# zchuning/repo

Hardware: AMD Instinct MI355X
Metric: world-model+imagine updates/sec (B=50,L=50,64x64x3) (higher is better)
Workload: dtype f32

## Files before the change

### repo_amd/csrc/conv.hip

```cpp
#include <stdlib.h>

#include <algorithm>
#include <type_traits>

#include "igemm.h"
#include "dconv.h"
#include "uconv.h"
#include "dconv_up.h"
#include "bconv.h"
#include "buconv.h"
#include "bwgrad.h"
#include "bdec4.h"
#include "twgrad.h"
#include "tconv_up.h"
#include "tconv_down.h"


namespace repo {

static thread_local int t_bconv_enabled = 1;

template <int CB_, int CS_, int HB_, int KS_>
struct Geo {
  static constexpr int CB = CB_, CS = CS_, HB = HB_, WB = HB_, KS = KS_;
// ... 201 lines not shown
  __shared__ float red[16][64];
  const int total = Mrows * (Ncols + 1) + (tkk > 0 ? 2 * tcb : 0);
  const int o = threadIdx.x & 63, gw = threadIdx.x >> 6;
  const int i = blockIdx.x * 64 + o;
  for (int g = gw; g < 16; g += SLAB_REDUCE_WAVES) {
    float s0 = 0.f, s1 = 0.f, s2 = 0.f, s3 = 0.f;
    if (i < total) {
      int z = g;
      for (; z + 48 < splits; z += 64) {
        s0 += slab[(size_t)z * total + i];
        s1 += slab[(size_t)(z + 16) * total + i];
        s2 += slab[(size_t)(z + 32) * total + i];
        s3 += slab[(size_t)(z + 48) * total + i];
      }
      for (; z < splits; z += 16) s0 += slab[(size_t)z * total + i];
    }
    red[g][o] = (s0 + s1) + (s2 + s3);
  }
  __syncthreads();
  const int g = gw;
  if (g == 0 && i < total) {
    float s = 0.f;
#pragma unroll
    for (int q = 0; q < 16; ++q) s += red[q][o];
    int m = i / (Ncols + 1), n = i % (Ncols + 1);
    if (tkk > 0) {
      const int body = Mrows * Ncols;
      if (i >= body + Mrows) {
        const int c = i - body - Mrows;
        if (dbig && c < tcb) {
          float s2 = 0.f;
#pragma unroll
          for (int q = 0; q < 16; ++q) s2 += red[q][o + tcb];
          dbig[c] = accumulate ? dbig[c] + (s + s2) : s + s2;
        }
        return;
      }
      if (i < body) m = (i / tcb) % Mrows, n = (i % tcb) * tkk + i / (tcb * Mrows);
      else m = i - body, n = Ncols;
    }
    if (n < Ncols) {
      float* p = dw + (size_t)m * Ncols + n;
      *p = accumulate ? *p + s : s;
    } else if (db) {
      db[m] = accumulate ? db[m] + s : s;
    }
  }
}

__global__ void partial_sum_rows_kernel(const float* __restrict__ parts, int n, float* __restrict__ out, float scale,
                                        int accumulate) {
  __shared__ float red[16];
  const float* row = parts + (size_t)blockIdx.x * n;
  float s = 0.f;
  for (int i = threadIdx.x; i < n; i += blockDim.x) s += row[i];
  s = block_sum(s, red);
  if (threadIdx.x == 0) out[blockIdx.x] = accumulate ? out[blockIdx.x] + scale * s : scale * s;
}

__global__ void partial_sum_kernel(const float* __restrict__ parts, int n, float* __restrict__ out, int accumulate) {
  __shared__ float red[16];
  float s = 0.f;
  for (int i = threadIdx.x; i < n; i += blockDim.x) s += parts[i];
  s = block_sum(s, red);
  if (threadIdx.x == 0) *out = accumulate ? *out + s : s;
}

__global__ void channel_sum_kernel(const float* __restrict__ x, int nimg, int C, int P, int imgs_per_split,
                                   float* __restrict__ parts) {
  __shared__ float red[16];
  const int c = blockIdx.x, s = blockIdx.y;
  const int i0 = s * imgs_per_split, i1 = min(nimg, i0 + imgs_per_split);
  const int nt = blockDim.x;
  const int dq = nt / P, dr = nt % P;
  int img = i0 + (int)threadIdx.x / P, p = (int)threadIdx.x % P;
  float a0 = 0.f, a1 = 0.f;
  const size_t cstride = (size_t)C * P;
  const float* base = x + (size_t)c * P;
  while (img < i1) {
    a0 += base[img * cstride + p];
    p += dr;
    img += dq;
    if (p >= P) {
      p -= P;
      ++img;
    }
    if (img >= i1) break;
    a1 += base[img * cstride + p];
    p += dr;
    img += dq;
    if (p >= P) {
      p -= P;
      ++img;
    }
  }
  const float acc = block_sum(a0 + a1, red);
  if (threadIdx.x == 0) parts[s * C + c] = acc;
}
__global__ void channel_sum_final_kernel(const float* __restrict__ parts, int splits, int C, float* __restrict__ out,
                                         int accumulate) {
  const int lane = threadIdx.x & 63;
  const int c = blockIdx.x * (blockDim.x >> 6) + (threadIdx.x >> 6);
  if (c >= C) return;
  float s = 0.f;
  for (int z = lane; z < splits; z += 64) s += parts[z * C + c];
  s = wave_sum(s);
  if (lane == 0) out[c] = accumulate ? out[c] + s : s;
}

__global__ void relu_mask_kernel(int64_t n, const float* __restrict__ dy, const float* __restrict__ h,
                                 float* __restrict__ y) {
  const int64_t stride = (int64_t)gridDim.x * blockDim.x;
  for (int64_t i = (int64_t)blockIdx.x * blockDim.x + threadIdx.x; i < n; i += stride) y[i] = h[i] > 0.f ? dy[i] : 0.f;
}

template <class G>
struct DTileFor;
template <> struct DTileFor<GEnc1> { using Down = DTile<32, 512, 3, 1, 8>; using Wgrad = WTile<32, 64, 1, 2, 1, 4, 2>; static constexpr int WGT = 3072; };
template <> struct DTileFor<GEnc2> { using Down = DTile<64, 128, 2, 2, 2>; using Wgrad = WTile<64, 128, 2, 2, 1, 7, 2>; static constexpr int WGT = 768; };
template <> struct DTileFor<GEnc3> { using Down = DTile<128, 128, 2, 2, 2>; using Wgrad = WTile<64, 128, 2, 2, 2, 6>; static constexpr int WGT = 1024; };
template <> struct DTileFor<GEnc4> { using Down = DTile<32, 64, 2, 1, 2>; using Wgrad = WTile<64, 128, 2, 2, 8, 2>; static constexpr int WGT = 768; };
template <> struct DTileFor<GDec2> { using Down = DTile<128, 128, 4, 2, 4, 1>; using Wgrad = WTile<64, 128, 2, 2, 4, 5>; static constexpr int WGT = 1536; };
template <> struct DTileFor<GDec3> { using Down = DTile<64, 128, 2, 2, 2>; using Wgrad = WTile<64, 128, 2, 2, 1, 7>; static constexpr int WGT = 2048; };
template <> struct DTileFor<GDec4> { using Down = DTile<32, 256, 3, 1, 8>; using Wgrad = WTile<32, 128, 1, 4, 1, 2>; static constexpr int WGT = 1536; };
template <> struct DTileFor<GX1> { using Down = DTile<32, 512, 3, 1, 8>;  using Wgrad = WTile<32, 64, 1, 2, 1, 2, 2>; static constexpr int WGT = 3072; };
template <> struct DTileFor<GX2> { using Down = DTile<64, 128, 2, 2, 2>;  using Wgrad = WTile<64, 128, 2, 2, 1, 3, 2>; static constexpr int WGT = 1536; };
template <> struct DTileFor<GX3> { using Down = DTile<128, 128, 2, 2, 2>; using Wgrad = WTile<64, 128, 2, 2, 1, 7>; static constexpr int WGT = 1024; };
template <> struct DTileFor<GX4> { using Down = DTile<64, 128, 2, 2, 2>;  using Wgrad = WTile<64, 128, 2, 2, 2, 6>; static constexpr int WGT = 1024; };
template <> struct DTileFor<GY4> { using Down = DTile<32, 256, 2, 1, 4>;  using Wgrad = WTile<32, 128, 1, 4, 1, 2>; static constexpr int WGT = 1536; };
template <> struct DTileFor<GT4> { using Down = DTile<32, 256, 3, 1, 8>;  using Wgrad = WTile<32, 128, 1, 4, 1, 2>; static constexpr int WGT = 1536; };
template <> struct DTileFor<GY5> { using Down = DTile<32, 512, 3, 1, 8>;  using Wgrad = WTile<32, 64, 1, 2, 1, 2>; static constexpr int WGT = 1536; };

template <class G> struct DLatTile { using type = typename DTileFor<G>::Down; };
template <> struct DLatTile<GEnc2> { using type = DTile<32, 128, 4, 1, 4>; };
template <> struct DLatTile<GEnc3> { using type = DTile<32, 128, 8, 1, 4>; };
template <> struct DLatTile<GEnc4> { using type = DTile<32, 128, 8, 1, 4>; };

struct NoBTile {};
template <class G> struct BDownFor { using type = NoBTile; };
template <> struct BDownFor<GDec3> { using type = BTile<64, 256, 2, 1, 4>; };
template <> struct BDownFor<GEnc3> { using type = BTile<128, 128, 4, 2, 2>; };
template <> struct BDownFor<GEnc4> { using type = BTile<128, 64, 4, 2, 2>; };
template <> struct BDownFor<GEnc2> { using type = BTile<64, 256, 4, 1, 4>; };
template <> struct BDownFor<GDec2> { using type = BTile<64, 128, 2, 1, 4>; };
template <class G> constexpr bool kBDown = !std::is_same<typename BDownFor<G>::type, NoBTile>::value;
template <class G> struct BDownU8For { using type = NoBTile; };
template <> struct BDownU8For<GEnc1> { using type = BTile<32, 512, 4, 1, 8>; };
template <class G> constexpr bool kBDownU8 = !std::is_same<typename BDownU8For<G>::type, NoBTile>::value;
template <class G, class BigT>
constexpr bool kBDownT = std::is_same<BigT, float>::value ? kBDown<G> : kBDownU8<G>;
template <class G, class BigT>
using BDownTile = typename std::conditional<std::is_same<BigT, float>::value, typename BDownFor<G>::type, typename BDownU8For<G>::type>::type;

template <class G, class BigT = float>
static bool bconv_down_on(int64_t nimg) {
  if constexpr (kBDownT<G, BigT>) return t_bconv_enabled && nimg * (int64_t)G::PS > 512;
  return false;
}
template <class G, class BigT = float>
static size_t bconv_pack_bytes() {
  if constexpr (kBDownT<G, BigT>) {
    typedef BPack<G, BDownTile<G, BigT>> P;
    return ((std::is_same<BigT, float>::value ? P::BYTES : P::BYTES_U8) + 255) & ~(size_t)255;
  }
  return 0;
}

template <class G, class BigT = float>
static long conv_down_tiles(int64_t nimg) {
  const long px = nimg * (long)G::PS;
  long bn = px <= 512 ? DLatTile<G>::type::BN : DTileFor<G>::Down::BN;
  if constexpr (kBDownT<G, BigT>)
    if (bconv_down_on<G, BigT>(nimg)) bn = BDownTile<G, BigT>::BN;
  return (px + bn - 1) / bn;
}

template <class G, class BigT>
static int conv_down_t(int64_t nimg, const BigT* big, const float* w, const float* bias, float* small, int epi,
                       const float* aux, float* dbias, int accumulate_dbias, unsigned char* cmask, void* ws,
                       size_t ws_bytes, hipStream_t s) {
  if (cmask && G::CS % 4 != 0) return REPO_E_BADARG;
  if (nimg * (int64_t)G::CB * G::PB >= kMaxBufElems || nimg * (int64_t)G::CS * G::PS >= kMaxBufElems) return REPO_E_SHAPE;
  bool bf = false;
  size_t pack_bytes = 0;
  if constexpr (kBDownT<G, BigT>) {
    pack_bytes = bconv_pack_bytes<G, BigT>();
    bf = bconv_down_on<G, BigT>(nimg) && ws && ws_bytes >= pack_bytes + (dbias ? (size_t)conv_down_tiles<G, BigT>(nimg) * G::CS * sizeof(float) : 0);
    if (!bf) pack_bytes = 0;
  }
  long tiles = conv_down_tiles<G, BigT>(nimg);
  if constexpr (kBDownT<G, BigT>)
    if (!bf && bconv_down_on<G, BigT>(nimg)) {
      const long px = nimg * (long)G::PS;
      tiles = (px + DTileFor<G>::Down::BN - 1) / DTileFor<G>::Down::BN;
    }
  if (dbias && (!ws || ws_bytes < pack_bytes + (size_t)tiles * G::CS * sizeof(float))) return REPO_E_WS_TOO_SMALL;
  float* parts = dbias ? (float*)((char*)ws + pack_bytes) : nullptr;
  DownArgs a{big, w, bias, aux, small, (int)nimg, epi, (unsigned)(nimg * G::CB * G::PB * sizeof(BigT)),
             (unsigned)(G::CS * G::CB * G::KK * sizeof(float)), parts, cmask};
  int rc;
#ifndef TCD_DISABLE
  if constexpr (std::is_same<G, GDec3>::value && std::is_same<BigT, float>::value) {
    if (bf && (epi == REPO_EPI_NONE || epi == REPO_EPI_MUL_DRELU) && !bias && !dbias && !cmask && nimg >= 32 &&
        pack_bytes >= TcdGeo::PACK_BYTES)
      return launch_tconv_down<TcdGeo>(a, w, (char*)ws, s);
  }
#ifndef TCD_NO_ENC2
  if constexpr (std::is_same<G, GEnc2>::value && std::is_same<BigT, float>::value) {
    if (bf && epi == REPO_EPI_RELU && !dbias && nimg >= 32 && pack_bytes >= TcdGeoE2::PACK_BYTES)
      return launch_tconv_down<TcdGeoE2>(a, w, (char*)ws, s);
  }
#endif
#endif
  if constexpr (kBDownT<G, BigT>) {
    if (bf) rc = launch_bconv_down<G, BDownTile<G, BigT>, BigT>(a, w, (char*)ws, s);
    else rc = (nimg * (int64_t)G::PS <= 512) ? launch_dconv_down<G, BigT, typename DLatTile<G>::type>(a, s)
                                            : launch_dconv_down<G, BigT, typename DTileFor<G>::Down>(a, s);
  } else {
    rc = (nimg * (int64_t)G::PS <= 512) ? launch_dconv_down<G, BigT, typename DLatTile<G>::type>(a, s)
                                        : launch_dconv_down<G, BigT, typename DTileFor<G>::Down>(a, s);
  }
  if (rc || !dbias) return rc;
  hipLaunchKernelGGL(channel_sum_final_kernel, dim3(cdiv(G::CS, 4)), dim3(256), 0, s, (const float*)parts, (int)tiles,
                     (int)G::CS, dbias, accumulate_dbias);
  REPO_CHECK_LAUNCH();
  return REPO_OK;
}

template <class G> struct UConf { using type = void; };
template <> struct UConf<GDec3> { using type = SConf<GDec3, 1, 6>; };
template <> struct UConf<GEnc2> { using type = SConf<GEnc2, 1, 8>; };
template <> struct UConf<GDec2> { using type = SConf<GDec2, 5, 2>; };
template <> struct UConf<GEnc3> { using type = SConf<GEnc3, 4, 2>; };
template <> struct UConf<GEnc4> { using type = SConf<GEnc4, 8, 1>; };
template <> struct UConf<GX3> { using type = SConf<GX3, 1, 2>; };
template <> struct UConf<GX4> { using type = SConf<GX4, 4, 1>; };

struct NoTile {};
template <class G> struct UpDirect { using type = NoTile; };
template <> struct UpDirect<GEnc2> { using type = NoTile; };
template <> struct UpDirect<GEnc3> { using type = NoTile; };
template <> struct UpDirect<GEnc4> { using type = NoTile; };
template <> struct UpDirect<GDec2> { using type = NoTile; };
template <> struct UpDirect<GDec3> { using type = NoTile; };
template <> struct UpDirect<GX2> { using type = DTile<128, 128, 8, 2, 4>; };
template <> struct UpDirect<GX3> { using type = NoTile; };
template <> struct UpDirect<GX4> { using type = NoTile; };
template <> struct UpDirect<GY4> { using type = DTile<64, 256, 4, 2, 4>; };
template <> struct UpDirect<GT4> { using type = DTile<32, 256, 4, 1, 8>; };
template <class G> constexpr bool kUpDirect = !std::is_same<typename UpDirect<G>::type, NoTile>::value;

template <class G> struct BUConf { using type = void; };
template <> struct BUConf<GDec3> { using type = BSConf<GDec3, 1, 4>; };
template <> struct BUConf<GEnc2> { using type = BSConf<GEnc2, 1, 4>; };
template <> struct BUConf<GEnc3> { using type = BSConf<GEnc3, 4, 4>; };
template <> struct BUConf<GEnc4> { using type = BSConf<GEnc4, 8, 2>; };
template <> struct BUConf<GDec2> { using type = BSConf<GDec2, 5, 4>; };
template <class G>
static bool buconv_on() {
  if constexpr (!std::is_void<typename BUConf<G>::type>::value) return t_bconv_enabled != 0;
  return false;
}

template <class G>
static size_t conv_up_ws_scatter() {
  using C = typename UConf<G>::type;
  using BC = typename BUConf<G>::type;
  if constexpr (kUpDirect<G>) return UpGeo<G>::PACK_FLOATS * sizeof(float);
  else if constexpr (std::is_void<C>::value) return 0;
  else if constexpr (!std::is_void<BC>::value) return BC::PACK_BYTES > C::PACK_FLOATS * sizeof(float) ? BC::PACK_BYTES : C::PACK_FLOATS * sizeof(float);
  else return C::PACK_FLOATS * sizeof(float);
}
template <class G> constexpr bool kTconvUp = false;
#ifndef TCU_DISABLE
template <> constexpr bool kTconvUp<GEnc2> = true;
#endif
template <class G>
static size_t conv_up_tcu_off() { return (conv_up_ws_scatter<G>() + 255) & ~(size_t)255; }
template <class G>
static size_t conv_up_ws_bytes() {
  if constexpr (kTconvUp<G>) return conv_up_tcu_off<G>() + kTcuPackBytes;
  return conv_up_ws_scatter<G>();
}

template <class G>
static int conv_up_pack_t(const float* w, void* ws, size_t ws_bytes, hipStream_t s) {
  using UC = typename UConf<G>::type;
  using BC = typename BUConf<G>::type;
  if constexpr (kTconvUp<G>) {
    if (buconv_on<G>()) {
      if (!ws || ws_bytes < conv_up_ws_bytes<G>()) return REPO_E_WS_TOO_SMALL;
      const int rc = launch_tconv_up_pack(w, (char*)ws + conv_up_tcu_off<G>(), s);
      if (rc) return rc;
    }
  }
  if constexpr (!std::is_void<BC>::value)
    if (buconv_on<G>()) return launch_buconv_pack<G, BC>(w, ws, ws_bytes, s);
  if constexpr (kUpDirect<G>) return launch_dconv_up_pack<G>(w, ws, ws_bytes, s);
  else if constexpr (!std::is_void<UC>::value) return launch_uconv_pack<G, UC>(w, ws, ws_bytes, s);
  else return REPO_OK;
}

template <class G>
static int conv_up_t(int64_t nimg, const float* small, const float* w, const float* bias, float* big, int epi,
                     const float* aux, int packed, void* ws, size_t ws_bytes, hipStream_t s) {
  if (nimg * (int64_t)G::CB * G::PB >= kMaxBufElems || nimg * (int64_t)G::CS * G::PS >= kMaxBufElems) return REPO_E_SHAPE;
  using UC = typename UConf<G>::type;
  using BC = typename BUConf<G>::type;
  if (epi == REPO_EPI_MUL_CMASK && (kUpDirect<G> || std::is_void<UC>::value || G::CB % 4 != 0)) return REPO_E_BADARG;
  if (epi == REPO_EPI_FILM_RELU && (kUpDirect<G> || std::is_void<UC>::value)) return REPO_E_BADARG;
  if constexpr (kTconvUp<G>) {
    const bool epi_ok = epi == REPO_EPI_NONE || epi == REPO_EPI_MUL_DRELU || epi == REPO_EPI_MUL_CMASK;
    if (buconv_on<G>() && epi_ok && nimg >= 4 && ws && ws_bytes >= conv_up_ws_bytes<G>()) {
      char* pack = (char*)ws + conv_up_tcu_off<G>();
      if (!packed) {
        const int rc = launch_tconv_up_pack(w, pack, s);
        if (rc) return rc;
      }
      return launch_tconv_up(small, pack, bias, aux, big, nimg, epi, s);
    }
  }
  if constexpr (!std::is_void<BC>::value)
    if (buconv_on<G>()) return launch_buconv_scatter<G, BC>(small, w, bias, aux, big, nimg, epi, packed, ws, ws_bytes, s);
  if constexpr (kUpDirect<G>) {
    return launch_dconv_up<G, typename UpDirect<G>::type>(small, w, bias, aux, big, nimg, epi, packed, ws, ws_bytes, s);
  } else if constexpr (!std::is_void<UC>::value) {
    return launch_uconv_scatter<G, UC>(small, w, bias, aux, big, nimg, epi, packed, ws, ws_bytes, s);
  } else {
    static_assert(G::KS % 2 == 0, "the gather engine pairs horizontally adjacent output pixels");
    ConvUpMergedOp<G, float, 0> op{small, w, bias, aux, big, (int)nimg, epi, nullptr, nullptr, nullptr, 0.f, 0.f};
    if constexpr (G::CB < 8) return launch_igemm<T32x256>(op, 4 * G::CB, nimg * (int64_t)op.NY * op.NX, 1, s);
    else return launch_igemm<T64x128>(op, 4 * G::CB, nimg * (int64_t)op.NY * op.NX, 1, s);
  }
}

template <class G>
static int dwgrad_ips(int64_t nimg) {
  using T = typename DTileFor<G>::Wgrad;
  const long tiles = ((G::CS + T::BM - 1) / T::BM) * ((G::CB * G::KK + T::BN - 1) / T::BN);
  long want = (DTileFor<G>::WGT + tiles - 1) / tiles;
  long ips = (nimg + want - 1) / want;
  const long min_ips = T::GI * ((G::PS >= 512) ? 1 : (G::PS >= 64 ? 2 : 4));
  if (ips < min_ips) ips = min_ips;
  ips = (ips + T::GI - 1) / T::GI * T::GI;
  return (int)ips;
}
template <class G>
static int dwgrad_splits(int64_t nimg) {
  const long ips = dwgrad_ips<G>(nimg);
  return (int)((nimg + ips - 1) / ips);
}
template <class G>
static size_t wgrad_ws_bytes(int64_t nimg) {
  return (size_t)dwgrad_splits<G>(nimg) * G::CS * (G::CB * G::KK + 1) * sizeof(float);
}

static void launch_conv_slab_reduce(const float* ws, int splits, int cs, int nw, float* dw, float* db, int accumulate,
                                    hipStream_t s) {
  const int total = cs * (nw + 1);
  if (splits >= 64 && total <= 65536) {
    hipLaunchKernelGGL(conv_slab_reduce_wave_kernel, dim3(cdiv(total, 64)), dim3(64 * SLAB_REDUCE_WAVES), 0, s, ws, splits, cs, nw, dw, db,
                       accumulate, 0, 0, (float*)nullptr);
  } else {
// ... 345 lines not shown
```

### repo_amd/csrc/tconv_down.h

```cpp
#pragma once
#include "bgemm.h"
#include "dconv.h"
#include "twgrad.h"

namespace repo {

template <int KS_, int WB_, int WS_, int GST_, int NTL_>
struct TcdGeoT {
  static constexpr int CB = 32, CS = 64, WB = WB_, HB = WB_, WS = WS_, PS = WS_ * WS_, PB = WB_ * WB_, KS = KS_, KK = KS_ * KS_;
  static_assert(KS % 2 == 0 && WS == (WB - KS) / 2 + 1 && HB <= 32, "even kernel, stride 2, at most 32 rows (the staging items)");
  static constexpr int CC = 8;
  static constexpr int NCH = CB / CC;
  static constexpr int NST = KK / 4;
  static constexpr int GST = GST_, NGR = NST / GST;
  static constexpr int XH = (WB + 1) / 2, PIXB = 16;
  static constexpr int PO = 256, ROWB = PO + XH * PIXB;
  static_assert(XH * PIXB <= PO, "a column-parity plane of a row fits 256 B");
  static constexpr int KP = KS / 2;
  static constexpr int tap_of(int s, int kg) { return ((2 * s + (kg >> 1)) / KP) * KS + 2 * ((2 * s + (kg >> 1)) % KP) + (kg & 1); }
  static constexpr int SLOTSTEP = (2 * ROWB / PIXB) % 16;
  static constexpr int PPLANE = HB * ROWB, PBUF = 3 * PPLANE;
  static constexpr int WPL = CS * 4 * 16;
  static constexpr int WSTEP = 3 * WPL, WGRP = GST * WSTEP;
  static constexpr int LDS_BYTES = 2 * PBUF + 2 * WGRP;
  static constexpr int NTL = NTL_;
  static constexpr int W_PER = WGRP / 16 / 256;
  static constexpr int QPR = (WB + 3) / 4, P_PER = 2;
  static_assert(WGRP % (16 * 256) == 0 && QPR == 8 && NST % GST == 0 && NCH % 2 == 0 && NGR <= 3 && NGR >= P_PER, "staging shares");
  static constexpr size_t PACK_BYTES = (size_t)NCH * NST * WSTEP;
};
using TcdGeo = TcdGeoT<6, 30, 13, 3, 6>;
using TcdGeoE2 = TcdGeoT<4, 31, 14, 2, 7>;
constexpr size_t kTcdPackBytes = TcdGeo::PACK_BYTES;

template <class T>
__global__ __launch_bounds__(256) void tconv_down_pack_kernel(const float* w, char* pack) {
  const int i = blockIdx.x * 256 + threadIdx.x;
  if (i >= T::NCH * T::NST * T::CS * 4) return;
  const int kg = i & 3, cs = (i >> 2) % T::CS, st = (i >> 2) / T::CS;
  const int c = st / T::NST, tap = T::tap_of(st % T::NST, kg);
  float v[8];
#pragma unroll
  for (int j = 0; j < 8; ++j) v[j] = w[((size_t)cs * T::CB + T::CC * c + j) * T::KK + tap];
  unsigned pl[3][4];
#pragma unroll
  for (int e = 0; e < 4; ++e) bg_split3(v[2 * e], v[2 * e + 1], pl[0][e], pl[1][e], pl[2][e]);
  char* dst = pack + (size_t)st * T::WSTEP + ((cs >> 4) * 64 + kg * 16 + (cs & 15)) * 16;
#pragma unroll
  for (int q = 0; q < 3; ++q) *reinterpret_cast<u32x4s*>(dst + q * T::WPL) = u32x4s{pl[q][0], pl[q][1], pl[q][2], pl[q][3]};
}

template <class T, int KEPI>
__global__ __launch_bounds__(512) void tconv_down_kernel(DownArgs p) {
  extern __shared__ __attribute__((aligned(16))) char td_lds[];
  char* const Pb = td_lds;
  char* const Wr = td_lds + 2 * T::PBUF;
  const int tid = threadIdx.x;
  const int wid = __builtin_amdgcn_readfirstlane(tid >> 6);
  const int nloc = (p.nimg - (int)blockIdx.x + (int)gridDim.x - 1) / (int)gridDim.x;
  if (nloc <= 0) return;
  const int nchunks = nloc * T::NCH;

  if (wid < 4) {
    __builtin_amdgcn_s_setprio(2);
    const int lane = tid & 63;
    const int mh = wid & 1, nh = wid >> 1;
    const int ln = lane & 15, kg = lane >> 4;
    int pxs[T::NTL], pfirst = 0;
#pragma unroll
    for (int t = 0; t < T::NTL; ++t) pxs[t] = -1;
    {
      int cnt = 0;
#pragma unroll
      for (int sy = T::WS - 1; sy >= 0; --sy) {
        const int sx = (ln - T::SLOTSTEP * sy) & 15;
        if (sx < T::WS) pfirst = T::WS * sy + sx;
      }
#pragma unroll
      for (int sy = 0; sy < T::WS; ++sy) {
        const int sx = (ln - T::SLOTSTEP * sy) & 15;
        const int idx = cnt - T::NTL * nh;
#pragma unroll
        for (int t = 0; t < T::NTL; ++t)
          if (sx < T::WS && idx == t) pxs[t] = T::WS * sy + sx;
        cnt += sx < T::WS ? 1 : 0;
      }
    }
    int nbase[T::NTL];
#pragma unroll
    for (int t = 0; t < T::NTL; ++t) {
      const int px = pxs[t] < 0 ? pfirst : pxs[t];
      const int sy = px / T::WS, sx = px - sy * T::WS;
      nbase[t] = 2 * sy * T::ROWB + sx * T::PIXB;
    }
    int toff[T::NST];
#pragma unroll
    for (int s = 0; s < T::NST; ++s) {
      const int pr = 2 * s + (kg >> 1), ky = pr / T::KP, kx = 2 * (pr - T::KP * ky) + (kg & 1);
      toff[s] = ky * T::ROWB + (kx & 1) * T::PO + (kx >> 1) * T::PIXB;
    }
    const int abase = 2 * mh * 1024 + lane * 16;

    f32x4 acc[2][T::NTL];
#pragma unroll
    for (int m = 0; m < 2; ++m)
#pragma unroll
      for (int t = 0; t < T::NTL; ++t) acc[m][t] = f32x4{0.f, 0.f, 0.f, 0.f};

    const __amdgpu_buffer_rsrc_t rout = make_rsrc(p.out, 4u * (unsigned)p.nimg * T::CS * T::PS);
    const __amdgpu_buffer_rsrc_t raux = make_rsrc(KEPI == REPO_EPI_MUL_DRELU ? p.aux : p.out, 4u * (unsigned)p.nimg * T::CS * T::PS);

    unsigned eoff[T::NTL];
#pragma unroll
    for (int t = 0; t < T::NTL; ++t) {
      eoff[t] = (4u * (unsigned)((32 * mh + 4 * kg) * T::PS + max(pxs[t], 0))) | ((unsigned)(pxs[t] >> 31) & kOobOffset);
    }
    float av[2][T::NTL][4];
    float bv[2][4];
#pragma unroll
    for (int m = 0; m < 2; ++m)
#pragma unroll
      for (int r = 0; r < 4; ++r) bv[m][r] = (KEPI == REPO_EPI_RELU && p.bias) ? p.bias[32 * mh + 16 * m + 4 * kg + r] : 0.f;

    lds_barrier();
    int ph = 0;
    for (int cc = 0; cc < nchunks; ++cc) {
      const char* Pl = Pb + (cc & 1) * T::PBUF;
      const unsigned ibase = 4u * (unsigned)(((int)blockIdx.x + (cc / T::NCH) * (int)gridDim.x) * T::CS * T::PS);
      if (KEPI == REPO_EPI_MUL_DRELU && (cc & (T::NCH - 1)) == T::NCH - 1) {
#pragma unroll
        for (int t = 0; t < T::NTL; ++t)
#pragma unroll
          for (int m = 0; m < 2; ++m)
#pragma unroll
            for (int r = 0; r < 4; ++r)
              av[m][t][r] = __builtin_bit_cast(float, __builtin_amdgcn_raw_buffer_load_b32(raux, eoff[t] + ibase + 4u * (unsigned)((16 * m + r) * T::PS), 0, 0));
      }
      bg_bf16x8 fa[2][2][3], fb[3][3];
#pragma unroll
      for (int g = 0; g < T::NGR; ++g) {
        const char* Wl = Wr + (ph & 1) * T::WGRP;
        auto load_a = [&](bg_bf16x8(&fa)[2][3], int k) __attribute__((always_inline)) {
#pragma unroll
          for (int m = 0; m < 2; ++m)
#pragma unroll
            for (int q = 0; q < 3; ++q)
              fa[m][q] = *reinterpret_cast<const bg_bf16x8*>(Wl + k * T::WSTEP + q * T::WPL + abase + m * 1024);
        };
        auto load_b = [&](bg_bf16x8(&fb)[3], int s, int t) __attribute__((always_inline)) {
#pragma unroll
          for (int q = 0; q < 3; ++q) fb[q] = *reinterpret_cast<const bg_bf16x8*>(Pl + q * T::PPLANE + nbase[t] + toff[s]);
        };
        load_a(fa[0], 0);
        if (g == 0) {
          load_b(fb[0], 0, 0);
          load_b(fb[1], 0, 1);
        }
        constexpr int NIT = T::GST * T::NTL;
#pragma unroll
        for (int it = 0; it < NIT; ++it) {
          const int k = it / T::NTL, t = it % T::NTL;
          if (it + 2 < NIT) load_b(fb[(it + 2) % 3], g * T::GST + (it + 2) / T::NTL, (it + 2) % T::NTL);
          if (t == 0 && k + 1 < T::GST) load_a(fa[(k + 1) & 1], k + 1);
          __builtin_amdgcn_sched_barrier(0);
          constexpr int PA[6] = {1, 0, 2, 0, 1, 0}, PB[6] = {1, 2, 0, 1, 0, 0};
#pragma unroll
          for (int pr = 0; pr < 6; ++pr)
#pragma unroll
            for (int m = 0; m < 2; ++m)
#ifdef TCD_NO_MFMA
              acc[m][t][0] += __builtin_bit_cast(float, (int)fa[k & 1][m][PA[pr]][0] + (int)fb[it % 3][PB[pr]][0]);
#else
              acc[m][t] = __builtin_amdgcn_mfma_f32_16x16x32_bf16(fa[k & 1][m][PA[pr]], fb[it % 3][PB[pr]], acc[m][t], 0, 0, 0);
#endif
          __builtin_amdgcn_sched_barrier(0);
        }
        if (g + 1 < T::NGR) {
          load_b(fb[0], (g + 1) * T::GST, 0);
          load_b(fb[1], (g + 1) * T::GST, 1);
        }
        lds_barrier();
        ++ph;
      }
#ifndef TCD_NO_EPI
      if ((cc & (T::NCH - 1)) == T::NCH - 1)
#else
      if (cc == nchunks - 1)
#endif
      {
        const int img = (int)blockIdx.x + (cc / T::NCH) * (int)gridDim.x;
#pragma unroll
        for (int t = 0; t < T::NTL; ++t)
#pragma unroll
          for (int m = 0; m < 2; ++m) {
            unsigned bits = 0;
#pragma unroll
            for (int r = 0; r < 4; ++r) {
              float x = acc[m][t][r];
              if (KEPI == REPO_EPI_MUL_DRELU) x = av[m][t][r] > 0.f ? x : 0.f;
              if (KEPI == REPO_EPI_RELU) {
                x = fmaxf(x + bv[m][r], 0.f);
                bits |= (x > 0.f ? 1u : 0u) << r;
              }
              __builtin_amdgcn_raw_buffer_store_b32(__builtin_bit_cast(unsigned, x), rout, eoff[t] + ibase + 4u * (unsigned)((16 * m + r) * T::PS), 0, 0);
              acc[m][t][r] = 0.f;
            }
            if (KEPI == REPO_EPI_RELU && p.cmask && pxs[t] >= 0)
              p.cmask[((size_t)img * (T::CS / 4) + 8 * mh + 4 * m + kg) * T::PS + pxs[t]] = (unsigned char)bits;
          }
      }
    }
  } else {
    const int t_ = tid - 256;
    const __amdgpu_buffer_rsrc_t rbg = make_rsrc(p.big, p.big_bytes), rw = make_rsrc(p.w, (unsigned)T::PACK_BYTES);
    f32x4 rwv[2][T::W_PER], rpv[2][T::P_PER][4];
    using I0 = std::integral_constant<int, 0>;
    using I1 = std::integral_constant<int, 1>;
    auto wload = [&](auto sc, int gi) __attribute__((always_inline)) {
      constexpr int S = decltype(sc)::value;
      const unsigned base = (unsigned)(gi % (T::NCH * T::NGR)) * (unsigned)T::WGRP;
#pragma unroll
      for (int i = 0; i < T::W_PER; ++i) rwv[S][i] = VecLoad<4>::load(rw, base + 16u * (unsigned)(t_ + 256 * i));
    };
    auto wstore = [&](auto sc, int gi) __attribute__((always_inline)) {
      constexpr int S = decltype(sc)::value;
      char* Wl = Wr + (gi & 1) * T::WGRP;
#pragma unroll
      for (int i = 0; i < T::W_PER; ++i) *reinterpret_cast<f32x4*>(Wl + 16 * (t_ + 256 * i)) = rwv[S][i];
    };
    auto x0_of = [](int q) { return T::WB % 2 == 0 ? min(4 * q, T::WB - 4) : 4 * q; };
    auto pload = [&](auto sc, int cc) __attribute__((always_inline)) {
      constexpr int S = decltype(sc)::value;
      const int img = (int)blockIdx.x + (cc / T::NCH) * (int)gridDim.x, c = cc & (T::NCH - 1);
      const unsigned dead_c = (unsigned)((nchunks - 1 - cc) >> 31);
#pragma unroll
      for (int i = 0; i < T::P_PER; ++i) {
        const int v = t_ + 256 * i, cq = v & 1, q = ((v >> 1) & 3) | (((v >> 4) & 1) << 2), row = ((v >> 3) & 1) | ((v >> 5) << 1);
        const unsigned dead = ((unsigned)((T::HB - 1 - row) >> 31) | dead_c) & kOobOffset;
        const int x0 = x0_of(q);
#pragma unroll
        for (int ch = 0; ch < 4; ++ch)
          rpv[S][i][ch] = VecLoad<4>::load(rbg, (4u * (unsigned)((img * T::CB + T::CC * c + 4 * cq + ch) * T::PB + row * T::WB + x0)) | dead);
      }
    };
    auto pstore = [&](auto sc, int cc, int i) __attribute__((always_inline)) {
      constexpr int S = decltype(sc)::value;
      char* Pl = Pb + (cc & 1) * T::PBUF;
      const int v = t_ + 256 * i, cq = v & 1, q = ((v >> 1) & 3) | (((v >> 4) & 1) << 2), row = ((v >> 3) & 1) | ((v >> 5) << 1);
      if (row < T::HB) {
        const int x0 = x0_of(q);
        char* base = Pl + row * T::ROWB + (x0 >> 1) * T::PIXB + cq * 8;
#pragma unroll
        for (int e = 0; e < 4; ++e) {
          unsigned a1, a2, a3, b1, b2, b3;
          tw_split3(rpv[S][i][0][e], rpv[S][i][1][e], a1, a2, a3);
          tw_split3(rpv[S][i][2][e], rpv[S][i][3][e], b1, b2, b3);
          char* dst = base + (e & 1) * T::PO + (e >> 1) * T::PIXB;
          *reinterpret_cast<bg_u32x2*>(dst) = bg_u32x2{a1, b1};
          *reinterpret_cast<bg_u32x2*>(dst + T::PPLANE) = bg_u32x2{a2, b2};
          *reinterpret_cast<bg_u32x2*>(dst + 2 * T::PPLANE) = bg_u32x2{a3, b3};
        }
      }
    };

    pload(I0{}, 0);
    wload(I0{}, 0);
    pstore(I0{}, 0, 0);
    pstore(I0{}, 0, 1);
    wstore(I0{}, 0);
    wload(I1{}, 1);
    wload(I0{}, 2);
    pload(I1{}, 1);
    pload(I0{}, 2);
    lds_barrier();
    auto phase = [&](auto pc, auto gc, int cc) __attribute__((always_inline)) {
      constexpr int P = decltype(pc)::value, g = decltype(gc)::value;
      constexpr int SW = (T::NGR * P + g + 1) & 1, SP = (P + 1) & 1;
      const int gi = T::NGR * cc + g;
#ifndef TCD_NO_STAGE
      wstore(std::integral_constant<int, SW>{}, gi + 1);
      wload(std::integral_constant<int, SW>{}, gi + 3);
      if constexpr (g < T::P_PER) pstore(std::integral_constant<int, SP>{}, cc + 1, g);
      if constexpr (g == T::P_PER - 1) pload(std::integral_constant<int, SP>{}, cc + 3);
#endif
      lds_barrier();
    };
    auto chunk = [&](auto pc, int cc) __attribute__((always_inline)) {
      phase(pc, std::integral_constant<int, 0>{}, cc);
      if constexpr (T::NGR > 1) phase(pc, std::integral_constant<int, 1>{}, cc);
      if constexpr (T::NGR > 2) phase(pc, std::integral_constant<int, 2>{}, cc);
    };
    for (int cc = 0; cc < nchunks; cc += 2) {
      chunk(I0{}, cc);
      chunk(I1{}, cc + 1);
    }
  }
}

template <class T, int KEPI>
inline int launch_tconv_down_k(const DownArgs& a, int grid, hipStream_t s) {
  static_assert(T::LDS_BYTES <= 160 * 1024, "tconv_down: LDS");
  hipError_t e = hipFuncSetAttribute((const void*)tconv_down_kernel<T, KEPI>, hipFuncAttributeMaxDynamicSharedMemorySize, T::LDS_BYTES);
  if (e != hipSuccess) return (int)e;
  hipLaunchKernelGGL((tconv_down_kernel<T, KEPI>), dim3((unsigned)grid), dim3(512), T::LDS_BYTES, s, a);
  e = hipGetLastError();
  return e == hipSuccess ? REPO_OK : (int)e;
}

template <class T>
inline int launch_tconv_down(const DownArgs& a, const float* w, char* pack, hipStream_t s) {
  hipLaunchKernelGGL(tconv_down_pack_kernel<T>, dim3((T::NCH * T::NST * T::CS * 4 + 255) / 256), dim3(256), 0, s, w, pack);
  hipError_t e = hipGetLastError();
  if (e != hipSuccess) return (int)e;
  DownArgs b = a;
  b.w = reinterpret_cast<const float*>(pack);
  static int cus = 0;
  if (!cus) {
    int dev = 0;
    if (hipGetDevice(&dev) != hipSuccess || hipDeviceGetAttribute(&cus, hipDeviceAttributeMultiprocessorCount, dev) != hipSuccess || cus <= 0)
      cus = 256;
  }
  const int grid = a.nimg < cus ? a.nimg : cus;
  if (a.epi == REPO_EPI_RELU) return launch_tconv_down_k<T, REPO_EPI_RELU>(b, grid, s);
  return a.epi == REPO_EPI_MUL_DRELU ? launch_tconv_down_k<T, REPO_EPI_MUL_DRELU>(b, grid, s) : launch_tconv_down_k<T, REPO_EPI_NONE>(b, grid, s);
}

}
```

Before: 170.1.

## Extend tconv_down MFMA path to deeper Dec2/Enc3 layers with multi-image blocks

Generalizes the bf16x3-split MFMA down-convolution kernel so it handles odd kernel sizes, larger channel counts and several small images per block, stacked in one LDS plane with split column-parity layout. It then routes the GDec2 and GEnc3 stride-2 convolutions to this kernel instead of the bconv path. Packing several small images per block is meant to fill MFMA tiles and reduce per-image overhead on the small deep layers. The cost is more complex indexing, zero-padded taps for odd kernels, and higher register and LDS pressure from the larger accumulator arrays.

```diff
diff --git a/repo_amd/csrc/conv.hip b/repo_amd/csrc/conv.hip
--- a/repo_amd/csrc/conv.hip
+++ b/repo_amd/csrc/conv.hip
@@ -377,6 +377,14 @@
 template <class G, class BigT>
 using BDownTile = typename std::conditional<std::is_same<BigT, float>::value, typename BDownFor<G>::type, typename BDownU8For<G>::type>::type;
 
+static_assert(TcdGeoD2::PACK_BYTES <= BPack<GDec2, BDownFor<GDec2>::type>::BYTES && TcdGeoE3::PACK_BYTES <= BPack<GEnc3, BDownFor<GEnc3>::type>::BYTES &&
+                  TcdGeo::PACK_BYTES <= BPack<GDec3, BDownFor<GDec3>::type>::BYTES &&
+                  TcdGeoE2::PACK_BYTES <= BPack<GEnc2, BDownFor<GEnc2>::type>::BYTES,
+              "tconv_down packs fit the bf16x6 pack's workspace slot");
+static_assert(TcdGeoD2::CB == GDec2::CB && TcdGeoD2::CS == GDec2::CS && TcdGeoD2::WB == GDec2::WB && TcdGeoD2::KS == GDec2::KS &&
+                  TcdGeoE3::CB == GEnc3::CB && TcdGeoE3::CS == GEnc3::CS && TcdGeoE3::WB == GEnc3::WB && TcdGeoE3::KS == GEnc3::KS,
+              "tconv_down geometries");
+
 template <class G, class BigT = float>
 static bool bconv_down_on(int64_t nimg) {
   if constexpr (kBDownT<G, BigT>) return t_bconv_enabled && nimg * (int64_t)G::PS > 512;
@@ -434,6 +442,17 @@
   if constexpr (std::is_same<G, GEnc2>::value && std::is_same<BigT, float>::value) {
     if (bf && epi == REPO_EPI_RELU && !dbias && nimg >= 32 && pack_bytes >= TcdGeoE2::PACK_BYTES)
       return launch_tconv_down<TcdGeoE2>(a, w, (char*)ws, s);
+  }
+#endif
+#ifndef TCD_NO_DEEP
+  if constexpr (std::is_same<G, GDec2>::value && std::is_same<BigT, float>::value) {
+    if (bf && (epi == REPO_EPI_NONE || epi == REPO_EPI_MUL_DRELU) && !bias && !dbias && !cmask && nimg >= 32 &&
+        pack_bytes >= TcdGeoD2::PACK_BYTES)
+      return launch_tconv_down<TcdGeoD2>(a, w, (char*)ws, s);
+  }
+  if constexpr (std::is_same<G, GEnc3>::value && std::is_same<BigT, float>::value) {
+    if (bf && epi == REPO_EPI_RELU && !dbias && nimg >= 32 && pack_bytes >= TcdGeoE3::PACK_BYTES)
+      return launch_tconv_down<TcdGeoE3>(a, w, (char*)ws, s);
   }
 #endif
 #endif
diff --git a/repo_amd/csrc/tconv_down.h b/repo_amd/csrc/tconv_down.h
--- a/repo_amd/csrc/tconv_down.h
+++ b/repo_amd/csrc/tconv_down.h
@@ -1,36 +1,61 @@
 #pragma once
+#include <utility>
 #include "bgemm.h"
 #include "dconv.h"
 #include "twgrad.h"
 
 namespace repo {
 
-template <int KS_, int WB_, int WS_, int GST_, int NTL_>
+template <int KS_, int WB_, int WS_, int GST_, int NTL_, int CB_ = 32, int CS_ = 64, int IPP_ = 1, int HBS_ = WB_, int MW_ = 2,
+          bool SPLIT_ = false>
 struct TcdGeoT {
-  static constexpr int CB = 32, CS = 64, WB = WB_, HB = WB_, WS = WS_, PS = WS_ * WS_, PB = WB_ * WB_, KS = KS_, KK = KS_ * KS_;
-  static_assert(KS % 2 == 0 && WS == (WB - KS) / 2 + 1 && HB <= 32, "even kernel, stride 2, at most 32 rows (the staging items)");
+  static constexpr int CB = CB_, CS = CS_, WB = WB_, HB = WB_, WS = WS_, PS = WS_ * WS_, PB = WB_ * WB_, KS = KS_, KK = KS_ * KS_;
+  static constexpr int IPP = IPP_, HBS = HBS_, NROWS = IPP_ * HBS_;
+  static constexpr bool SPLIT = SPLIT_;
+  static_assert(WS == (WB - KS) / 2 + 1 && HBS >= HB && (SPLIT || (IPP == 1 && HB <= 32 && KS % 2 == 0)), "stride 2; geometry");
   static constexpr int CC = 8;
   static constexpr int NCH = CB / CC;
-  static constexpr int NST = KK / 4;
+  static constexpr int KP = (KS + 1) / 2, NPAIR = KS * KP;
+  static constexpr int NST = (NPAIR + 1) / 2;
   static constexpr int GST = GST_, NGR = NST / GST;
   static constexpr int XH = (WB + 1) / 2, PIXB = 16;
-  static constexpr int PO = 256, ROWB = PO + XH * PIXB;
-  static_assert(XH * PIXB <= PO, "a column-parity plane of a row fits 256 B");
-  static constexpr int KP = KS / 2;
-  static constexpr int tap_of(int s, int kg) { return ((2 * s + (kg >> 1)) / KP) * KS + 2 * ((2 * s + (kg >> 1)) % KP) + (kg & 1); }
-  static constexpr int SLOTSTEP = (2 * ROWB / PIXB) % 16;
-  static constexpr int PPLANE = HB * ROWB, PBUF = 3 * PPLANE;
+  static constexpr int ROWB = SPLIT ? XH * PIXB : 256 + XH * PIXB;
+  static constexpr int PO = SPLIT ? (NROWS * ROWB + 255) / 256 * 256 : 256;
+  static_assert(XH * PIXB <= 256, "a column-parity plane of a row fits 256 B");
+  static constexpr int pair_of(int s, int kg) { return (2 * s + (kg >> 1)) < NPAIR ? 2 * s + (kg >> 1) : 0; }
+  static constexpr int ky_of(int s, int kg) { return pair_of(s, kg) / KP; }
+  static constexpr int kx_of(int s, int kg) { return 2 * (pair_of(s, kg) % KP) + (kg & 1); }
+  static constexpr bool tap_ok(int s, int kg) { return 2 * s + (kg >> 1) < NPAIR && kx_of(s, kg) < KS; }
+  static constexpr int tap_of(int s, int kg) { return ky_of(s, kg) * KS + kx_of(s, kg); }
+  static constexpr int row_slot(int row) { return (row * (ROWB / PIXB)) % 16; }
+  static constexpr int PPLANE = SPLIT ? PO + NROWS * ROWB : NROWS * ROWB, PBUF = 3 * PPLANE;
   static constexpr int WPL = CS * 4 * 16;
   static constexpr int WSTEP = 3 * WPL, WGRP = GST * WSTEP;
   static constexpr int LDS_BYTES = 2 * PBUF + 2 * WGRP;
+  static constexpr int MW = MW_, NW = 4 / MW_, MT = CS / (16 * MW_);
   static constexpr int NTL = NTL_;
   static constexpr int W_PER = WGRP / 16 / 256;
-  static constexpr int QPR = (WB + 3) / 4, P_PER = 2;
-  static_assert(WGRP % (16 * 256) == 0 && QPR == 8 && NST % GST == 0 && NCH % 2 == 0 && NGR <= 3 && NGR >= P_PER, "staging shares");
+  static constexpr int QPR = (WB + 3) / 4, NITEM = IPP * HB * QPR * 2;
+  static constexpr int P_PER = SPLIT ? (NITEM + 255) / 256 : 2;
+  static_assert(WGRP % (16 * 256) == 0 && (SPLIT || QPR == 8) && NST % GST == 0 && NCH % 2 == 0 && (NCH & (NCH - 1)) == 0 &&
+                    NGR >= P_PER && MW * NW == 4 && MT * 16 * MW == CS && GST * NTL >= 2,
+                "staging shares");
+  static constexpr int max_slot_count() {
+    int c[16] = {};
+    for (int i = 0; i < IPP; ++i)
+      for (int sy = 0; sy < WS; ++sy)
+        for (int sx = 0; sx < WS; ++sx) ++c[(row_slot(i * HBS + 2 * sy) + sx) % 16];
+    int m = 0;
+    for (int j = 0; j < 16; ++j) m = c[j] > m ? c[j] : m;
+    return m;
+  }
+  static_assert(max_slot_count() <= NW * NTL && WS <= 16, "pixel tiles");
   static constexpr size_t PACK_BYTES = (size_t)NCH * NST * WSTEP;
 };
 using TcdGeo = TcdGeoT<6, 30, 13, 3, 6>;
 using TcdGeoE2 = TcdGeoT<4, 31, 14, 2, 7>;
+using TcdGeoD2 = TcdGeoT<5, 13, 5, 1, 9, 64, 128, 5, 15, 4, true>;
+using TcdGeoE3 = TcdGeoT<4, 14, 6, 1, 13, 64, 128, 5, 15, 4, true>;
 constexpr size_t kTcdPackBytes = TcdGeo::PACK_BYTES;
 
 template <class T>
@@ -39,15 +64,21 @@
   if (i >= T::NCH * T::NST * T::CS * 4) return;
   const int kg = i & 3, cs = (i >> 2) % T::CS, st = (i >> 2) / T::CS;
   const int c = st / T::NST, tap = T::tap_of(st % T::NST, kg);
+  const bool ok = T::tap_ok(st % T::NST, kg);
   float v[8];
 #pragma unroll
-  for (int j = 0; j < 8; ++j) v[j] = w[((size_t)cs * T::CB + T::CC * c + j) * T::KK + tap];
+  for (int j = 0; j < 8; ++j) v[j] = ok ? w[((size_t)cs * T::CB + T::CC * c + j) * T::KK + tap] : 0.f;
   unsigned pl[3][4];
 #pragma unroll
   for (int e = 0; e < 4; ++e) bg_split3(v[2 * e], v[2 * e + 1], pl[0][e], pl[1][e], pl[2][e]);
   char* dst = pack + (size_t)st * T::WSTEP + ((cs >> 4) * 64 + kg * 16 + (cs & 15)) * 16;
 #pragma unroll
   for (int q = 0; q < 3; ++q) *reinterpret_cast<u32x4s*>(dst + q * T::WPL) = u32x4s{pl[q][0], pl[q][1], pl[q][2], pl[q][3]};
+}
+
+template <class F, int... G>
+__device__ __forceinline__ void tcd_for_each(std::integer_sequence<int, G...>, F&& f) {
+  (f(std::integral_constant<int, G>{}), ...);
 }
 
 template <class T, int KEPI>
@@ -57,14 +88,15 @@
   char* const Wr = td_lds + 2 * T::PBUF;
   const int tid = threadIdx.x;
   const int wid = __builtin_amdgcn_readfirstlane(tid >> 6);
-  const int nloc = (p.nimg - (int)blockIdx.x + (int)gridDim.x - 1) / (int)gridDim.x;
+  const int ngrp = (p.nimg + T::IPP - 1) / T::IPP;
+  const int nloc = (ngrp - (int)blockIdx.x + (int)gridDim.x - 1) / (int)gridDim.x;
   if (nloc <= 0) return;
   const int nchunks = nloc * T::NCH;
 
   if (wid < 4) {
     __builtin_amdgcn_s_setprio(2);
     const int lane = tid & 63;
-    const int mh = wid & 1, nh = wid >> 1;
+    const int mh = wid % T::MW, nh = wid / T::MW;
     const int ln = lane & 15, kg = lane >> 4;
     int pxs[T::NTL], pfirst = 0;
 #pragma unroll
@@ -72,38 +104,40 @@
     {
       int cnt = 0;
 #pragma unroll
-      for (int sy = T::WS - 1; sy >= 0; --sy) {
-        const int sx = (ln - T::SLOTSTEP * sy) & 15;
-        if (sx < T::WS) pfirst = T::WS * sy + sx;
-      }
-#pragma unroll
-      for (int sy = 0; sy < T::WS; ++sy) {
-        const int sx = (ln - T::SLOTSTEP * sy) & 15;
+      for (int r = T::IPP * T::WS - 1; r >= 0; --r) {
+        const int i = r / T::WS, sy = r - i * T::WS;
+        const int sx = (ln - T::row_slot(i * T::HBS + 2 * sy)) & 15;
+        if (sx < T::WS) pfirst = T::PS * i + T::WS * sy + sx;
+      }
+#pragma unroll
+      for (int r = 0; r < T::IPP * T::WS; ++r) {
+        const int i = r / T::WS, sy = r - i * T::WS;
+        const int sx = (ln - T::row_slot(i * T::HBS + 2 * sy)) & 15;
         const int idx = cnt - T::NTL * nh;
 #pragma unroll
         for (int t = 0; t < T::NTL; ++t)
-          if (sx < T::WS && idx == t) pxs[t] = T::WS * sy + sx;
+          if (sx < T::WS && idx == t) pxs[t] = T::PS * i + T::WS * sy + sx;
         cnt += sx < T::WS ? 1 : 0;
       }
     }
     int nbase[T::NTL];
 #pragma unroll
     for (int t = 0; t < T::NTL; ++t) {
-      const int px = pxs[t] < 0 ? pfirst : pxs[t];
-      const int sy = px / T::WS, sx = px - sy * T::WS;
-      nbase[t] = 2 * sy * T::ROWB + sx * T::PIXB;
+      const int n = pxs[t] < 0 ? pfirst : pxs[t];
+      const int i = n / T::PS, px = n - i * T::PS, sy = px / T::WS, sx = px - sy * T::WS;
+      nbase[t] = (i * T::HBS + 2 * sy) * T::ROWB + sx * T::PIXB;
     }
     int toff[T::NST];
 #pragma unroll
     for (int s = 0; s < T::NST; ++s) {
-      const int pr = 2 * s + (kg >> 1), ky = pr / T::KP, kx = 2 * (pr - T::KP * ky) + (kg & 1);
+      const int ky = T::ky_of(s, kg), kx = T::kx_of(s, kg);
       toff[s] = ky * T::ROWB + (kx & 1) * T::PO + (kx >> 1) * T::PIXB;
     }
-    const int abase = 2 * mh * 1024 + lane * 16;
-
-    f32x4 acc[2][T::NTL];
-#pragma unroll
-    for (int m = 0; m < 2; ++m)
+    const int abase = T::MT * mh * 1024 + lane * 16;
+
+    f32x4 acc[T::MT][T::NTL];
+#pragma unroll
+    for (int m = 0; m < T::MT; ++m)
 #pragma unroll
       for (int t = 0; t < T::NTL; ++t) acc[m][t] = f32x4{0.f, 0.f, 0.f, 0.f};
 
@@ -111,38 +145,47 @@
     const __amdgpu_buffer_rsrc_t raux = make_rsrc(KEPI == REPO_EPI_MUL_DRELU ? p.aux : p.out, 4u * (unsigned)p.nimg * T::CS * T::PS);
 
     unsigned eoff[T::NTL];
+    int pimg[T::NTL];
 #pragma unroll
     for (int t = 0; t < T::NTL; ++t) {
-      eoff[t] = (4u * (unsigned)((32 * mh + 4 * kg) * T::PS + max(pxs[t], 0))) | ((unsigned)(pxs[t] >> 31) & kOobOffset);
-    }
-    float av[2][T::NTL][4];
-    float bv[2][4];
-#pragma unroll
-    for (int m = 0; m < 2; ++m)
-#pragma unroll
-      for (int r = 0; r < 4; ++r) bv[m][r] = (KEPI == REPO_EPI_RELU && p.bias) ? p.bias[32 * mh + 16 * m + 4 * kg + r] : 0.f;
+      const int n = max(pxs[t], 0), i = n / T::PS, px = n - i * T::PS;
+      pimg[t] = i;
+      eoff[t] = (4u * (unsigned)((i * T::CS + 16 * T::MT * mh + 4 * kg) * T::PS + px)) | ((unsigned)(pxs[t] >> 31) & kOobOffset);
+    }
+    float av[T::MT][T::NTL][4];
+    float bv[T::MT][4];
+#pragma unroll
+    for (int m = 0; m < T::MT; ++m)
+#pragma unroll
+      for (int r = 0; r < 4; ++r) bv[m][r] = (KEPI == REPO_EPI_RELU && p.bias) ? p.bias[16 * (T::MT * mh + m) + 4 * kg + r] : 0.f;
+    auto out_off = [&](int t, int grp) __attribute__((always_inline)) {
+      const unsigned o = eoff[t] + 4u * (unsigned)(grp * T::IPP * T::CS * T::PS);
+      return (T::IPP > 1 && grp * T::IPP + pimg[t] >= p.nimg) ? (o | kOobOffset) : o;
+    };
 
     lds_barrier();
     int ph = 0;
     for (int cc = 0; cc < nchunks; ++cc) {
       const char* Pl = Pb + (cc & 1) * T::PBUF;
-      const unsigned ibase = 4u * (unsigned)(((int)blockIdx.x + (cc / T::NCH) * (int)gridDim.x) * T::CS * T::PS);
-      if (KEPI == REPO_EPI_MUL_DRELU && (cc & (T::NCH - 1)) == T::NCH - 1) {
-#pragma unroll
-        for (int t = 0; t < T::NTL; ++t)
-#pragma unroll
-          for (int m = 0; m < 2; ++m)
+      const int grp = (int)blockIdx.x + (cc / T::NCH) * (int)gridDim.x;
+      if (KEPI == REPO_EPI_MUL_DRELU && (cc & (T::NCH - 1)) == T::NCH - 1 && !T::SPLIT) {
+#pragma unroll
+        for (int t = 0; t < T::NTL; ++t) {
+          const unsigned o = out_off(t, grp);
+#pragma unroll
+          for (int m = 0; m < T::MT; ++m)
 #pragma unroll
             for (int r = 0; r < 4; ++r)
-              av[m][t][r] = __builtin_bit_cast(float, __builtin_amdgcn_raw_buffer_load_b32(raux, eoff[t] + ibase + 4u * (unsigned)((16 * m + r) * T::PS), 0, 0));
-      }
-      bg_bf16x8 fa[2][2][3], fb[3][3];
+              av[m][t][r] = __builtin_bit_cast(float, __builtin_amdgcn_raw_buffer_load_b32(raux, o + 4u * (unsigned)((16 * m + r) * T::PS), 0, 0));
+        }
+      }
+      bg_bf16x8 fa[2][T::MT][3], fb[3][3];
 #pragma unroll
       for (int g = 0; g < T::NGR; ++g) {
         const char* Wl = Wr + (ph & 1) * T::WGRP;
-        auto load_a = [&](bg_bf16x8(&fa)[2][3], int k) __attribute__((always_inline)) {
-#pragma unroll
-          for (int m = 0; m < 2; ++m)
+        auto load_a = [&](bg_bf16x8(&fa)[T::MT][3], int k) __attribute__((always_inline)) {
+#pragma unroll
+          for (int m = 0; m < T::MT; ++m)
 #pragma unroll
             for (int q = 0; q < 3; ++q)
               fa[m][q] = *reinterpret_cast<const bg_bf16x8*>(Wl + k * T::WSTEP + q * T::WPL + abase + m * 1024);
@@ -154,7 +197,7 @@
         load_a(fa[0], 0);
         if (g == 0) {
           load_b(fb[0], 0, 0);
-          load_b(fb[1], 0, 1);
+          load_b(fb[1], 1 / T::NTL, 1 % T::NTL);
         }
         constexpr int NIT = T::GST * T::NTL;
 #pragma unroll
@@ -167,7 +210,7 @@
 #pragma unroll
           for (int pr = 0; pr < 6; ++pr)
 #pragma unroll
-            for (int m = 0; m < 2; ++m)
+            for (int m = 0; m < T::MT; ++m)
 #ifdef TCD_NO_MFMA
               acc[m][t][0] += __builtin_bit_cast(float, (int)fa[k & 1][m][PA[pr]][0] + (int)fb[it % 3][PB[pr]][0]);
 #else
@@ -177,7 +220,7 @@
         }
         if (g + 1 < T::NGR) {
           load_b(fb[0], (g + 1) * T::GST, 0);
-          load_b(fb[1], (g + 1) * T::GST, 1);
+          load_b(fb[1], (g + 1) * T::GST + 1 / T::NTL, 1 % T::NTL);
         }
         lds_barrier();
         ++ph;
@@ -188,11 +231,19 @@
       if (cc == nchunks - 1)
 #endif
       {
-        const int img = (int)blockIdx.x + (cc / T::NCH) * (int)gridDim.x;
-#pragma unroll
-        for (int t = 0; t < T::NTL; ++t)
-#pragma unroll
-          for (int m = 0; m < 2; ++m) {
+#pragma unroll
+        for (int t = 0; t < T::NTL; ++t) {
+          const unsigned o = out_off(t, grp);
+          const int img = grp * T::IPP + pimg[t], px = max(pxs[t], 0) - pimg[t] * T::PS;
+          if (KEPI == REPO_EPI_MUL_DRELU && T::SPLIT) {
+#pragma unroll
+            for (int m = 0; m < T::MT; ++m)
+#pragma unroll
+              for (int r = 0; r < 4; ++r)
+                av[m][t][r] = __builtin_bit_cast(float, __builtin_amdgcn_raw_buffer_load_b32(raux, o + 4u * (unsigned)((16 * m + r) * T::PS), 0, 0));
+          }
+#pragma unroll
+          for (int m = 0; m < T::MT; ++m) {
             unsigned bits = 0;
 #pragma unroll
             for (int r = 0; r < 4; ++r) {
@@ -202,12 +253,13 @@
                 x = fmaxf(x + bv[m][r], 0.f);
                 bits |= (x > 0.f ? 1u : 0u) << r;
               }
-              __builtin_amdgcn_raw_buffer_store_b32(__builtin_bit_cast(unsigned, x), rout, eoff[t] + ibase + 4u * (unsigned)((16 * m + r) * T::PS), 0, 0);
+              __builtin_amdgcn_raw_buffer_store_b32(__builtin_bit_cast(unsigned, x), rout, o + 4u * (unsigned)((16 * m + r) * T::PS), 0, 0);
               acc[m][t][r] = 0.f;
             }
-            if (KEPI == REPO_EPI_RELU && p.cmask && pxs[t] >= 0)
-              p.cmask[((size_t)img * (T::CS / 4) + 8 * mh + 4 * m + kg) * T::PS + pxs[t]] = (unsigned char)bits;
+            if (KEPI == REPO_EPI_RELU && p.cmask && pxs[t] >= 0 && img < p.nimg)
+              p.cmask[((size_t)img * (T::CS / 4) + 4 * (T::MT * mh + m) + kg) * T::PS + px] = (unsigned char)bits;
           }
+        }
       }
     }
   } else {
@@ -229,29 +281,47 @@
       for (int i = 0; i < T::W_PER; ++i) *reinterpret_cast<f32x4*>(Wl + 16 * (t_ + 256 * i)) = rwv[S][i];
     };
     auto x0_of = [](int q) { return T::WB % 2 == 0 ? min(4 * q, T::WB - 4) : 4 * q; };
+    auto item = [&](int v, int& cq, int& q, int& img, int& row) __attribute__((always_inline)) {
+      cq = v & 1;
+      if constexpr (T::SPLIT) {
+        q = (v >> 1) % T::QPR;
+        const int rr = (v >> 1) / T::QPR;
+        img = rr / T::HB;
+        row = rr - img * T::HB;
+      } else {
+        q = ((v >> 1) & 3) | (((v >> 4) & 1) << 2);
+        row = ((v >> 3) & 1) | ((v >> 5) << 1);
+        img = 0;
+      }
+    };
     auto pload = [&](auto sc, int cc) __attribute__((always_inline)) {
       constexpr int S = decltype(sc)::value;
-      const int img = (int)blockIdx.x + (cc / T::NCH) * (int)gridDim.x, c = cc & (T::NCH - 1);
+      const int grp = (int)blockIdx.x + (cc / T::NCH) * (int)gridDim.x, c = cc & (T::NCH - 1);
       const unsigned dead_c = (unsigned)((nchunks - 1 - cc) >> 31);
 #pragma unroll
       for (int i = 0; i < T::P_PER; ++i) {
-        const int v = t_ + 256 * i, cq = v & 1, q = ((v >> 1) & 3) | (((v >> 4) & 1) << 2), row = ((v >> 3) & 1) | ((v >> 5) << 1);
-        const unsigned dead = ((unsigned)((T::HB - 1 - row) >> 31) | dead_c) & kOobOffset;
+        int cq, q, img, row;
+        item(t_ + 256 * i, cq, q, img, row);
+        const int gimg = grp * T::IPP + img;
+        const unsigned dead = ((unsigned)((T::HB - 1 - row) >> 31) | (unsigned)((T::IPP - 1 - img) >> 31) |
+                               (unsigned)((p.nimg - 1 - gimg) >> 31) | dead_c) & kOobOffset;
         const int x0 = x0_of(q);
 #pragma unroll
         for (int ch = 0; ch < 4; ++ch)
-          rpv[S][i][ch] = VecLoad<4>::load(rbg, (4u * (unsigned)((img * T::CB + T::CC * c + 4 * cq + ch) * T::PB + row * T::WB + x0)) | dead);
+          rpv[S][i][ch] = VecLoad<4>::load(rbg, (4u * (unsigned)((gimg * T::CB + T::CC * c + 4 * cq + ch) * T::PB + row * T::WB + x0)) | dead);
       }
     };
     auto pstore = [&](auto sc, int cc, int i) __attribute__((always_inline)) {
       constexpr int S = decltype(sc)::value;
       char* Pl = Pb + (cc & 1) * T::PBUF;
-      const int v = t_ + 256 * i, cq = v & 1, q = ((v >> 1) & 3) | (((v >> 4) & 1) << 2), row = ((v >> 3) & 1) | ((v >> 5) << 1);
-      if (row < T::HB) {
+      int cq, q, img, row;
+      item(t_ + 256 * i, cq, q, img, row);
+      if (row < T::HB && img < T::IPP) {
         const int x0 = x0_of(q);
-        char* base = Pl + row * T::ROWB + (x0 >> 1) * T::PIXB + cq * 8;
+        char* base = Pl + (img * T::HBS + row) * T::ROWB + (x0 >> 1) * T::PIXB + cq * 8;
 #pragma unroll
         for (int e = 0; e < 4; ++e) {
+          if (T::SPLIT && (x0 >> 1) + (e >> 1) >= T::XH) continue;
           unsigned a1, a2, a3, b1, b2, b3;
           tw_split3(rpv[S][i][0][e], rpv[S][i][1][e], a1, a2, a3);
           tw_split3(rpv[S][i][2][e], rpv[S][i][3][e], b1, b2, b3);
@@ -265,8 +335,8 @@
 
     pload(I0{}, 0);
     wload(I0{}, 0);
-    pstore(I0{}, 0, 0);
-    pstore(I0{}, 0, 1);
+#pragma unroll
+    for (int i = 0; i < T::P_PER; ++i) pstore(I0{}, 0, i);
     wstore(I0{}, 0);
     wload(I1{}, 1);
     wload(I0{}, 2);
@@ -286,9 +356,7 @@
       lds_barrier();
     };
     auto chunk = [&](auto pc, int cc) __attribute__((always_inline)) {
-      phase(pc, std::integral_constant<int, 0>{}, cc);
-      if constexpr (T::NGR > 1) phase(pc, std::integral_constant<int, 1>{}, cc);
-      if constexpr (T::NGR > 2) phase(pc, std::integral_constant<int, 2>{}, cc);
+      tcd_for_each(std::make_integer_sequence<int, T::NGR>{}, [&](auto gc) __attribute__((always_inline)) { phase(pc, gc, cc); });
     };
     for (int cc = 0; cc < nchunks; cc += 2) {
       chunk(I0{}, cc);
@@ -320,7 +388,8 @@
     if (hipGetDevice(&dev) != hipSuccess || hipDeviceGetAttribute(&cus, hipDeviceAttributeMultiprocessorCount, dev) != hipSuccess || cus <= 0)
       cus = 256;
   }
-  const int grid = a.nimg < cus ? a.nimg : cus;
+  const int ngrp = (a.nimg + T::IPP - 1) / T::IPP;
+  const int grid = ngrp < cus ? ngrp : cus;
   if (a.epi == REPO_EPI_RELU) return launch_tconv_down_k<T, REPO_EPI_RELU>(b, grid, s);
   return a.epi == REPO_EPI_MUL_DRELU ? launch_tconv_down_k<T, REPO_EPI_MUL_DRELU>(b, grid, s) : launch_tconv_down_k<T, REPO_EPI_NONE>(b, grid, s);
 }
```

Result: no change. 168.4 (median of 2 runs) (-1.0%).
